# daisy9542/yolo-puncture

Hardware: AMD Instinct MI355X
Metric: images/sec (higher is better)
Workload: dtype bf16

## Files before the change

yolo-puncture_amd/csrc/conv_dwpw_stream.hip:

```cpp
#include "common.h"
#include <cstdlib>

namespace yp {

typedef __attribute__((ext_vector_type(8))) __bf16 bf16x8;
typedef __attribute__((ext_vector_type(4))) float f32x4;
typedef __attribute__((ext_vector_type(2))) float f32x2;
typedef __attribute__((address_space(3))) void lds_void;

constexpr int DS_TH = 8, DS_TW = 16;
constexpr int DS_C = 128;
constexpr int DS_HP = (DS_TH + 2) * (DS_TW + 2);
constexpr int DS_PIECES = 48;
constexpr int DS_HB = DS_PIECES * 1024;
constexpr int DS_AB = DS_TH * DS_TW * 256;

template <int N> __device__ __forceinline__ void ds_wait_vm() {
    static_assert(N >= 0 && N < 64, "vmcnt range");
    __builtin_amdgcn_s_waitcnt((N & 0xF) | (7 << 4) | (0xF << 8) | (((N >> 4) & 3) << 14));
}
__device__ __forceinline__ unsigned ds_lds_addr(const void* p) { return (unsigned)(size_t)(const __attribute__((address_space(3))) unsigned char*)p; }

template <int NW>
__global__ __launch_bounds__(NW * 64, 2) void conv_dwpw_stream_kernel(const DwPwParams p, const int tiles_h, const int tiles_w, const int num_tiles, const int G) {
    constexpr int RPW = DS_TH / NW;
    constexpr int NFW = 8 / NW;
    constexpr int NSLOT = NW == 8 ? 2 : 1;
    constexpr int NST = DS_TH * NFW;
    constexpr unsigned OOB = 0x80000000u;
    extern __shared__ __attribute__((aligned(1024))) unsigned char smem[];
    unsigned char* const Hs = smem;
    unsigned char* const As = smem + NSLOT * DS_HB;
    const int tid = threadIdx.x, lane = tid & 63;
    const int wave = __builtin_amdgcn_readfirstlane(tid >> 6);
    const int fr = lane & 15, fc = lane >> 4;

    const __amdgpu_buffer_rsrc_t xrs = __builtin_amdgcn_make_buffer_rsrc((void*)p.x, 0, (int)p.x_bytes, 0x00020000);
    const __amdgpu_buffer_rsrc_t wrs = __builtin_amdgcn_make_buffer_rsrc((void*)p.w_pw, 0, (int)p.wpw_bytes, 0x00020000);
    const __amdgpu_buffer_rsrc_t yrs = __builtin_amdgcn_make_buffer_rsrc((void*)p.y, 0, (int)p.y_bytes, 0x00020000);

    auto issue_tile = [&](int tile, int slot) {
        int t = tile;
        const int tw = t % tiles_w; t /= tiles_w;
        const int th = t % tiles_h;
        const int b = t / tiles_h;
        const int h0 = th * DS_TH - 1, w0 = tw * DS_TW - 1;
        unsigned char* const dst = Hs + slot * DS_HB;
#pragma unroll
        for (int j = 0; j < DS_PIECES / NW; ++j) {
            const int ii = wave + j * NW;
            const int s = ii * 64 + lane;
            const int hp = s >> 4, c = s & 15;
            const int hy = hp / (DS_TW + 2), hx = hp - hy * (DS_TW + 2);
            const int hi = h0 + hy, wi = w0 + hx;
            const bool ok = tile < num_tiles && hp < DS_HP && (unsigned)hi < (unsigned)p.H && (unsigned)wi < (unsigned)p.W;
            const unsigned voff = ok ? (unsigned)((((b * p.H + hi) * p.W + wi) * p.x_stride + p.x_coff + c * 8) * 2) : OOB;
            __builtin_amdgcn_raw_ptr_buffer_load_lds(xrs, (lds_void*)(dst + ii * 1024), 16, voff, 0, 0, 0);
        }
    };
    int tile = blockIdx.x;
    issue_tile(tile, 0);

    f32x2 wd[9], bd;
    {
        const unsigned* w32 = (const unsigned*)p.w_dw;
#pragma unroll
        for (int t = 0; t < 9; ++t) {
            const unsigned u = w32[t * (DS_C / 2) + lane];
            wd[t] = f32x2{__uint_as_float(u << 16), __uint_as_float(u & 0xffff0000u)};
        }
        bd = f32x2{p.b_dw[2 * lane], p.b_dw[2 * lane + 1]};
    }
    bf16x8 wreg[4][NFW];
    float bpw[NFW][4];
#pragma unroll
    for (int i = 0; i < NFW; ++i) {
#pragma unroll
        for (int ks = 0; ks < 4; ++ks) {
            const unsigned voff = (unsigned)((((wave * NFW + i) * 16 + fr) * p.Kpad + (ks >> 1) * 64 + fc * 16 + (ks & 1) * 8) * 2);
            const __attribute__((ext_vector_type(4))) unsigned v = __builtin_amdgcn_raw_buffer_load_b128(wrs, voff, 0, 0);
            wreg[ks][i] = __builtin_bit_cast(bf16x8, v);
        }
#pragma unroll
        for (int r = 0; r < 4; ++r) { const int co = (wave * NFW + i) * 16 + fc * 4 + r; bpw[i][r] = (co < p.Cout) ? p.b_pw[co] : 0.f; }
    }
    ds_wait_vm<0>();
#pragma unroll
    for (int t = 0; t < 9; ++t) asm volatile("" : "+v"(wd[t]));
    asm volatile("" : "+v"(bd));
#pragma unroll
    for (int i = 0; i < NFW; ++i) {
#pragma unroll
        for (int ks = 0; ks < 4; ++ks) asm volatile("" : "+v"(wreg[ks][i]));
#pragma unroll
        for (int r = 0; r < 4; ++r) asm volatile("" : "+v"(bpw[i][r]));
    }

    const unsigned as_l = ds_lds_addr(As);
    for (int it = 0; tile < num_tiles; tile += G, ++it) {
        if (it == 0) ds_wait_vm<0>();
        else ds_wait_vm<NST>();
        __builtin_amdgcn_s_barrier();
        const int slot = NSLOT == 2 ? (it & 1) : 0;
        if (NSLOT == 2) issue_tile(tile + G, slot ^ 1);
        int t = tile;
        const int tw = t % tiles_w; t /= tiles_w;
        const int th = t % tiles_h;
        const int b = t / tiles_h;
#pragma unroll
        for (int rr = 0; rr < RPW; ++rr) {
            const int row = wave * RPW + rr;
            f32x2 win[3][3];
            auto rd = [&](int ky, int col) -> f32x2 {
                const unsigned u = *(const unsigned*)(Hs + slot * DS_HB + ((row + ky) * (DS_TW + 2) + col) * 256 + lane * 4);
                return f32x2{__uint_as_float(u << 16), __uint_as_float(u & 0xffff0000u)};
            };
#pragma unroll
            for (int ky = 0; ky < 3; ++ky) { win[ky][0] = rd(ky, 0); win[ky][1] = rd(ky, 1); }
#pragma unroll
            for (int x = 0; x < DS_TW; ++x) {
#pragma unroll
                for (int ky = 0; ky < 3; ++ky) win[ky][2] = rd(ky, x + 2);
                f32x2 a = bd;
#pragma unroll
                for (int ky = 0; ky < 3; ++ky)
#pragma unroll
                    for (int kx = 0; kx < 3; ++kx) a = __builtin_elementwise_fma(win[ky][kx], wd[ky * 3 + kx], a);
                if (p.act_dw == ACT_SILU) {
                    f32x2 e = a * -1.4426950408889634f;
                    e[0] = __builtin_amdgcn_exp2f(e[0]); e[1] = __builtin_amdgcn_exp2f(e[1]);
                    e = e + 1.0f;
                    e[0] = __builtin_amdgcn_rcpf(e[0]); e[1] = __builtin_amdgcn_rcpf(e[1]);
                    a = a * e;
                }
                __attribute__((aligned(4))) __bf16 o[2] = {(__bf16)a[0], (__bf16)a[1]};
                const int px = row * DS_TW + x;
                const unsigned dst = as_l + (unsigned)(px * 256 + (((lane >> 2) ^ (px & 15)) << 4) + (lane & 3) * 4);
                asm volatile("ds_write_b32 %0, %1" : : "v"(dst), "v"(*(const unsigned*)o) : "memory");
#pragma unroll
                for (int ky = 0; ky < 3; ++ky) { win[ky][0] = win[ky][1]; win[ky][1] = win[ky][2]; }
            }
        }
        asm volatile("s_waitcnt lgkmcnt(0)" ::: "memory");
        __builtin_amdgcn_s_barrier();
        if (NSLOT == 1) issue_tile(tile + G, 0);
        f32x4 acc[NFW][DS_TH];
#pragma unroll
        for (int i = 0; i < NFW; ++i)
#pragma unroll
            for (int f = 0; f < DS_TH; ++f) acc[i][f] = f32x4{bpw[i][0], bpw[i][1], bpw[i][2], bpw[i][3]};
#pragma unroll
        for (int ks = 0; ks < 4; ++ks) {
            const int ch = (ks >> 1) * 8 + fc * 2 + (ks & 1);
            bf16x8 xf[DS_TH];
#pragma unroll
            for (int f = 0; f < DS_TH; ++f) xf[f] = *(const bf16x8*)(As + (f * 16 + fr) * 256 + ((ch ^ fr) << 4));
#pragma unroll
            for (int i = 0; i < NFW; ++i)
#pragma unroll
                for (int f = 0; f < DS_TH; ++f) acc[i][f] = __builtin_amdgcn_mfma_f32_16x16x32_bf16(wreg[ks][i], xf[f], acc[i][f], 0, 0, 0);
        }
        const int wo = tw * DS_TW + fr;
#pragma unroll
        for (int i = 0; i < NFW; ++i) {
            const int co = (wave * NFW + i) * 16 + fc * 4;
#pragma unroll
            for (int f = 0; f < DS_TH; ++f) {
                const int ho = th * DS_TH + f;
                const bool ok = ho < p.H && wo < p.W && co < p.Cout;
                float v[4] = {acc[i][f][0], acc[i][f][1], acc[i][f][2], acc[i][f][3]};
                if (p.act_pw == ACT_SILU) silu4_packed(v);
                __attribute__((aligned(8))) __bf16 o[4] = {(__bf16)v[0], (__bf16)v[1], (__bf16)v[2], (__bf16)v[3]};
                const unsigned off = ok ? (unsigned)((((b * p.H + ho) * p.W + wo) * p.y_stride + p.y_coff + co) * 2) : OOB;
                __builtin_amdgcn_raw_buffer_store_b64(*(const __attribute__((ext_vector_type(2))) unsigned*)o, yrs, off, 0, 0);
            }
        }
    }
    ds_wait_vm<0>();
}

bool dwpw_stream_valid(const DwPwParams& p) {
    static const bool off = [] { const char* v = std::getenv("YOLOP_NO_DWPW_STREAM"); return v && *v == '1'; }();
    if (off || p.w3 || p.out_f32 || p.clk) return false;
    if (p.C != DS_C || p.Kpad != DS_C || p.Cout != 128) return false;
    if ((p.x_stride & 7) || (p.x_coff & 7) || (p.y_stride & 3) || (p.y_coff & 3)) return false;
    if (p.x_bytes >= (1ull << 31) || p.y_bytes >= (1ull << 31) || p.wpw_bytes >= (1ull << 31)) return false;
    if (p.act_dw != ACT_SILU && p.act_dw != ACT_NONE) return false;
    if (p.act_pw != ACT_SILU && p.act_pw != ACT_NONE) return false;
    return (long)((p.H + DS_TH - 1) / DS_TH * DS_TH) * ((p.W + DS_TW - 1) / DS_TW * DS_TW) * 2 <= (long)p.H * p.W * 3;
}

template <int NW>
static hipError_t launch_dwpw_stream_t(const DwPwParams& p, hipStream_t st) {
    const size_t sh = (size_t)(NW == 8 ? 2 : 1) * DS_HB + DS_AB;
    auto kern = conv_dwpw_stream_kernel<NW>;
    static bool attr = false;
    if (!attr) {
        hipError_t e = hipFuncSetAttribute((const void*)kern, hipFuncAttributeMaxDynamicSharedMemorySize, 160 * 1024);
        if (e != hipSuccess) return e;
        attr = true;
    }
    const int tiles_h = (p.H + DS_TH - 1) / DS_TH, tiles_w = (p.W + DS_TW - 1) / DS_TW;
    const int num_tiles = p.B * tiles_h * tiles_w;
    const int gmax = NW == 8 ? 256 : 512;
    const int G = num_tiles < gmax ? num_tiles : gmax;
    hipLaunchKernelGGL(kern, dim3((unsigned)G), dim3(NW * 64), sh, st, p, tiles_h, tiles_w, num_tiles, G);
    return hipGetLastError();
}

hipError_t launch_dwpw_stream(const DwPwParams& p, hipStream_t st) {
    if (!dwpw_stream_valid(p)) return hipErrorInvalidValue;
    static const bool one = [] { const char* v = std::getenv("YOLOP_DWPW_STREAM_ONE"); return v && *v == '1'; }();
    return one ? launch_dwpw_stream_t<8>(p, st) : launch_dwpw_stream_t<4>(p, st);
}

}
```

Measured before the change: 22390.

## Software-pipeline depthwise stage with paired LDS reads and templated activations

Restructures the depthwise loop into unrolled 4-column groups. Halo reads are issued one group ahead with ds_read2st64 pairs and explicit lgkmcnt waits, so LDS latency overlaps the FMAs. Write addresses become compile-time offsets on a precomputed base, and the activation types become template parameters so the runtime branches disappear. It also adds an optional s_memtime clock instrumentation path. In exchange it carries more registers for double-buffered raw reads, and it relies on hand-counted waitcnt values being correct.

```diff
diff --git a/yolo-puncture_amd/csrc/conv_dwpw_stream.hip b/yolo-puncture_amd/csrc/conv_dwpw_stream.hip
--- a/yolo-puncture_amd/csrc/conv_dwpw_stream.hip
+++ b/yolo-puncture_amd/csrc/conv_dwpw_stream.hip
@@ -1,11 +1,16 @@
 #include "common.h"
+#include <cstdio>
 #include <cstdlib>
+#include <utility>
+#include <vector>
 
 namespace yp {
 
 typedef __attribute__((ext_vector_type(8))) __bf16 bf16x8;
 typedef __attribute__((ext_vector_type(4))) float f32x4;
 typedef __attribute__((ext_vector_type(2))) float f32x2;
+typedef __attribute__((ext_vector_type(2))) __bf16 bf16x2;
+typedef __attribute__((ext_vector_type(2))) unsigned u32x2;
 typedef __attribute__((address_space(3))) void lds_void;
 
 constexpr int DS_TH = 8, DS_TW = 16;
@@ -13,6 +18,7 @@
 constexpr int DS_HP = (DS_TH + 2) * (DS_TW + 2);
 constexpr int DS_PIECES = 48;
 constexpr int DS_HB = DS_PIECES * 1024;
+static_assert(DS_HB % 1024 == 0, "the depthwise stage's write swizzle is one XOR into address bits 4..7: every halo slot and the operand tile behind them must start 1-KiB aligned");
 constexpr int DS_AB = DS_TH * DS_TW * 256;
 
 template <int N> __device__ __forceinline__ void ds_wait_vm() {
@@ -21,12 +27,35 @@
 }
 __device__ __forceinline__ unsigned ds_lds_addr(const void* p) { return (unsigned)(size_t)(const __attribute__((address_space(3))) unsigned char*)p; }
 
-template <int NW>
+template <int P0, int P1> __device__ __forceinline__ void ds_rd2px(u32x2& d, unsigned a) {
+    static_assert(P0 >= 0 && P1 < 256, "ds_read2st64 offset range");
+    asm volatile("ds_read2st64_b32 %0, %1 offset0:%2 offset1:%3" : "=v"(d) : "v"(a), "n"(P0), "n"(P1));
+}
+template <int OFF> __device__ __forceinline__ void ds_wr32(unsigned a, unsigned v) {
+    static_assert(OFF >= 0 && OFF < 65536, "ds_write offset range");
+    asm volatile("ds_write_b32 %0, %1 offset:%2" : : "v"(a), "v"(v), "n"(OFF));
+}
+template <int N, bool FIRST> __device__ __forceinline__ void ds_wait_lgkm(u32x2 (&r)[3][3]) {
+    static_assert(N >= 0 && N < 16, "lgkmcnt range");
+    if (FIRST)
+        asm volatile("s_waitcnt lgkmcnt(%9)" : "+v"(r[0][0]), "+v"(r[0][1]), "+v"(r[0][2]), "+v"(r[1][0]), "+v"(r[1][1]), "+v"(r[1][2]),
+                                               "+v"(r[2][0]), "+v"(r[2][1]), "+v"(r[2][2]) : "n"(N));
+    else
+        asm volatile("s_waitcnt lgkmcnt(%6)" : "+v"(r[0][1]), "+v"(r[0][2]), "+v"(r[1][1]), "+v"(r[1][2]), "+v"(r[2][1]), "+v"(r[2][2]) : "n"(N));
+}
+template <int... I, class F> __device__ __forceinline__ void ds_static_for(std::integer_sequence<int, I...>, F&& f) { (f(std::integral_constant<int, I>{}), ...); }
+__device__ __forceinline__ unsigned ds_pk_bf16(float a, float b) {
+    return __builtin_bit_cast(unsigned, __builtin_convertvector(f32x2{a, b}, bf16x2));
+}
+
+template <int NW, int ADW, int APW, bool CLK>
 __global__ __launch_bounds__(NW * 64, 2) void conv_dwpw_stream_kernel(const DwPwParams p, const int tiles_h, const int tiles_w, const int num_tiles, const int G) {
     constexpr int RPW = DS_TH / NW;
     constexpr int NFW = 8 / NW;
     constexpr int NSLOT = NW == 8 ? 2 : 1;
     constexpr int NST = DS_TH * NFW;
+    constexpr int CG = 4;
+    constexpr int NU = RPW * (DS_TW / CG);
     constexpr unsigned OOB = 0x80000000u;
     extern __shared__ __attribute__((aligned(1024))) unsigned char smem[];
     unsigned char* const Hs = smem;
@@ -38,6 +67,12 @@
     const __amdgpu_buffer_rsrc_t xrs = __builtin_amdgcn_make_buffer_rsrc((void*)p.x, 0, (int)p.x_bytes, 0x00020000);
     const __amdgpu_buffer_rsrc_t wrs = __builtin_amdgcn_make_buffer_rsrc((void*)p.w_pw, 0, (int)p.wpw_bytes, 0x00020000);
     const __amdgpu_buffer_rsrc_t yrs = __builtin_amdgcn_make_buffer_rsrc((void*)p.y, 0, (int)p.y_bytes, 0x00020000);
+
+    unsigned long long clk[5] = {0, 0, 0, 0, 0};
+    unsigned long long last = 0;
+    auto stamp = [&](int i) {
+        if (CLK) { const unsigned long long now = __builtin_amdgcn_s_memtime(); clk[i] += now - last; last = now; }
+    };
 
     auto issue_tile = [&](int tile, int slot) {
         int t = tile;
@@ -96,53 +131,81 @@
         for (int r = 0; r < 4; ++r) asm volatile("" : "+v"(bpw[i][r]));
     }
 
-    const unsigned as_l = ds_lds_addr(As);
+    const unsigned hs_l = ds_lds_addr(Hs) + (unsigned)(wave * RPW * (DS_TW + 2) * 256 + lane * 4);
+    const unsigned aw_l = ds_lds_addr(As) + (unsigned)(wave * RPW * DS_TW * 256 + ((lane >> 2) << 4) + (lane & 3) * 4);
+    if (CLK) last = __builtin_amdgcn_s_memtime();
     for (int it = 0; tile < num_tiles; tile += G, ++it) {
-        if (it == 0) ds_wait_vm<0>();
-        else ds_wait_vm<NST>();
+        ds_wait_vm<NST>();
         __builtin_amdgcn_s_barrier();
+        stamp(0);
         const int slot = NSLOT == 2 ? (it & 1) : 0;
+        const unsigned hs_t = hs_l + (unsigned)(slot * DS_HB);
+        u32x2 raw[2][3][3];
+        auto rd = [&](auto U) {
+            constexpr int u = decltype(U)::value, rr = u / (DS_TW / CG), c0 = (u % (DS_TW / CG)) * CG;
+            ds_static_for(std::make_integer_sequence<int, 3>{}, [&](auto KY) {
+                constexpr int ky = decltype(KY)::value, px = (rr + ky) * (DS_TW + 2) + c0;
+                if (c0 == 0) ds_rd2px<px, px + 1>(raw[u & 1][ky][0], hs_t);
+                ds_rd2px<px + 2, px + 3>(raw[u & 1][ky][1], hs_t);
+                ds_rd2px<px + 4, px + 5>(raw[u & 1][ky][2], hs_t);
+            });
+        };
+        rd(std::integral_constant<int, 0>{});
         if (NSLOT == 2) issue_tile(tile + G, slot ^ 1);
         int t = tile;
         const int tw = t % tiles_w; t /= tiles_w;
         const int th = t % tiles_h;
         const int b = t / tiles_h;
-#pragma unroll
-        for (int rr = 0; rr < RPW; ++rr) {
-            const int row = wave * RPW + rr;
-            f32x2 win[3][3];
-            auto rd = [&](int ky, int col) -> f32x2 {
-                const unsigned u = *(const unsigned*)(Hs + slot * DS_HB + ((row + ky) * (DS_TW + 2) + col) * 256 + lane * 4);
-                return f32x2{__uint_as_float(u << 16), __uint_as_float(u & 0xffff0000u)};
-            };
-#pragma unroll
-            for (int ky = 0; ky < 3; ++ky) { win[ky][0] = rd(ky, 0); win[ky][1] = rd(ky, 1); }
-#pragma unroll
-            for (int x = 0; x < DS_TW; ++x) {
-#pragma unroll
-                for (int ky = 0; ky < 3; ++ky) win[ky][2] = rd(ky, x + 2);
-                f32x2 a = bd;
-#pragma unroll
-                for (int ky = 0; ky < 3; ++ky)
-#pragma unroll
-                    for (int kx = 0; kx < 3; ++kx) a = __builtin_elementwise_fma(win[ky][kx], wd[ky * 3 + kx], a);
-                if (p.act_dw == ACT_SILU) {
-                    f32x2 e = a * -1.4426950408889634f;
-                    e[0] = __builtin_amdgcn_exp2f(e[0]); e[1] = __builtin_amdgcn_exp2f(e[1]);
-                    e = e + 1.0f;
-                    e[0] = __builtin_amdgcn_rcpf(e[0]); e[1] = __builtin_amdgcn_rcpf(e[1]);
-                    a = a * e;
-                }
-                __attribute__((aligned(4))) __bf16 o[2] = {(__bf16)a[0], (__bf16)a[1]};
-                const int px = row * DS_TW + x;
-                const unsigned dst = as_l + (unsigned)(px * 256 + (((lane >> 2) ^ (px & 15)) << 4) + (lane & 3) * 4);
-                asm volatile("ds_write_b32 %0, %1" : : "v"(dst), "v"(*(const unsigned*)o) : "memory");
-#pragma unroll
-                for (int ky = 0; ky < 3; ++ky) { win[ky][0] = win[ky][1]; win[ky][1] = win[ky][2]; }
+        f32x2 car[3][2];
+        ds_static_for(std::make_integer_sequence<int, NU>{}, [&](auto U) {
+            constexpr int u = decltype(U)::value, rr = u / (DS_TW / CG), c0 = (u % (DS_TW / CG)) * CG;
+            constexpr bool first = c0 == 0, nfirst = (u + 1) % (DS_TW / CG) == 0;
+            if constexpr (u + 1 < NU) rd(std::integral_constant<int, u + 1>{});
+            ds_wait_lgkm<(u > 0 ? CG : 0) + (u + 1 < NU ? (nfirst ? 9 : 6) : 0), first>(raw[u & 1]);
+            f32x2 win[3][CG + 2];
+#pragma unroll
+            for (int ky = 0; ky < 3; ++ky) {
+#pragma unroll
+                for (int q = first ? 0 : 1; q < 3; ++q)
+#pragma unroll
+                    for (int h = 0; h < 2; ++h) {
+                        const unsigned v = raw[u & 1][ky][q][h];
+                        win[ky][2 * q + h] = f32x2{__uint_as_float(v << 16), __uint_as_float(v & 0xffff0000u)};
+                    }
+                if (!first) { win[ky][0] = car[ky][0]; win[ky][1] = car[ky][1]; }
+                car[ky][0] = win[ky][CG]; car[ky][1] = win[ky][CG + 1];
             }
-        }
+            f32x2 a[CG];
+#pragma unroll
+            for (int j = 0; j < CG; ++j) a[j] = bd;
+#pragma unroll
+            for (int ky = 0; ky < 3; ++ky)
+#pragma unroll
+                for (int kx = 0; kx < 3; ++kx)
+#pragma unroll
+                    for (int j = 0; j < CG; ++j) a[j] = __builtin_elementwise_fma(win[ky][j + kx], wd[ky * 3 + kx], a[j]);
+            if (ADW == ACT_SILU) {
+                f32x2 e[CG];
+#pragma unroll
+                for (int j = 0; j < CG; ++j) e[j] = a[j] * -1.4426950408889634f;
+#pragma unroll
+                for (int j = 0; j < CG; ++j) { e[j][0] = __builtin_amdgcn_exp2f(e[j][0]); e[j][1] = __builtin_amdgcn_exp2f(e[j][1]); }
+#pragma unroll
+                for (int j = 0; j < CG; ++j) e[j] = e[j] + 1.0f;
+#pragma unroll
+                for (int j = 0; j < CG; ++j) { e[j][0] = __builtin_amdgcn_rcpf(e[j][0]); e[j][1] = __builtin_amdgcn_rcpf(e[j][1]); }
+#pragma unroll
+                for (int j = 0; j < CG; ++j) a[j] = a[j] * e[j];
+            }
+            ds_static_for(std::make_integer_sequence<int, CG>{}, [&](auto J) {
+                constexpr int x = c0 + decltype(J)::value;
+                ds_wr32<(rr * DS_TW + x) * 256>(aw_l ^ (unsigned)(x << 4), ds_pk_bf16(a[decltype(J)::value][0], a[decltype(J)::value][1]));
+            });
+        });
         asm volatile("s_waitcnt lgkmcnt(0)" ::: "memory");
+        stamp(1);
         __builtin_amdgcn_s_barrier();
+        stamp(2);
         if (NSLOT == 1) issue_tile(tile + G, 0);
         f32x4 acc[NFW][DS_TH];
 #pragma unroll
@@ -160,6 +223,7 @@
 #pragma unroll
                 for (int f = 0; f < DS_TH; ++f) acc[i][f] = __builtin_amdgcn_mfma_f32_16x16x32_bf16(wreg[ks][i], xf[f], acc[i][f], 0, 0, 0);
         }
+        stamp(3);
         const int wo = tw * DS_TW + fr;
 #pragma unroll
         for (int i = 0; i < NFW; ++i) {
@@ -169,14 +233,16 @@
                 const int ho = th * DS_TH + f;
                 const bool ok = ho < p.H && wo < p.W && co < p.Cout;
                 float v[4] = {acc[i][f][0], acc[i][f][1], acc[i][f][2], acc[i][f][3]};
-                if (p.act_pw == ACT_SILU) silu4_packed(v);
-                __attribute__((aligned(8))) __bf16 o[4] = {(__bf16)v[0], (__bf16)v[1], (__bf16)v[2], (__bf16)v[3]};
+                if (APW == ACT_SILU) silu4_packed(v);
                 const unsigned off = ok ? (unsigned)((((b * p.H + ho) * p.W + wo) * p.y_stride + p.y_coff + co) * 2) : OOB;
-                __builtin_amdgcn_raw_buffer_store_b64(*(const __attribute__((ext_vector_type(2))) unsigned*)o, yrs, off, 0, 0);
+                __builtin_amdgcn_raw_buffer_store_b64(u32x2{ds_pk_bf16(v[0], v[1]), ds_pk_bf16(v[2], v[3])}, yrs, off, 0, 0);
             }
         }
+        stamp(4);
     }
     ds_wait_vm<0>();
+    if (CLK && lane == 0)
+        for (int i = 0; i < 5; ++i) p.clk[((size_t)blockIdx.x * NW + wave) * 5 + i] = clk[i];
 }
 
 bool dwpw_stream_valid(const DwPwParams& p) {
@@ -190,10 +256,10 @@
     return (long)((p.H + DS_TH - 1) / DS_TH * DS_TH) * ((p.W + DS_TW - 1) / DS_TW * DS_TW) * 2 <= (long)p.H * p.W * 3;
 }
 
-template <int NW>
+template <int NW, int ADW, int APW>
 static hipError_t launch_dwpw_stream_t(const DwPwParams& p, hipStream_t st) {
     const size_t sh = (size_t)(NW == 8 ? 2 : 1) * DS_HB + DS_AB;
-    auto kern = conv_dwpw_stream_kernel<NW>;
+    auto kern = conv_dwpw_stream_kernel<NW, ADW, APW, false>;
     static bool attr = false;
     if (!attr) {
         hipError_t e = hipFuncSetAttribute((const void*)kern, hipFuncAttributeMaxDynamicSharedMemorySize, 160 * 1024);
@@ -204,14 +270,51 @@
     const int num_tiles = p.B * tiles_h * tiles_w;
     const int gmax = NW == 8 ? 256 : 512;
     const int G = num_tiles < gmax ? num_tiles : gmax;
+    static const bool clocks = [] { const char* v = std::getenv("YOLOP_DWPW_STREAM_CLOCKS"); return v && *v == '1'; }();
+    if (clocks) {
+        hipStreamCaptureStatus cap = hipStreamCaptureStatusNone;
+        hipError_t e = hipStreamIsCapturing(st, &cap);
+        if (e != hipSuccess) return e;
+        if (cap != hipStreamCaptureStatusNone) return hipErrorStreamCaptureUnsupported;
+        auto kclk = conv_dwpw_stream_kernel<NW, ADW, APW, true>;
+        e = hipFuncSetAttribute((const void*)kclk, hipFuncAttributeMaxDynamicSharedMemorySize, 160 * 1024);
+        if (e != hipSuccess) return e;
+        DwPwParams q = p;
+        const size_t n = (size_t)G * NW * 5;
+        e = hipMalloc((void**)&q.clk, n * 8);
+        if (e != hipSuccess) return e;
+        std::vector<unsigned long long> h(n);
+        hipLaunchKernelGGL(kclk, dim3((unsigned)G), dim3(NW * 64), sh, st, q, tiles_h, tiles_w, num_tiles, G);
+        e = hipGetLastError();
+        if (e == hipSuccess) e = hipStreamSynchronize(st);
+        if (e == hipSuccess) e = hipMemcpy(h.data(), q.clk, n * 8, hipMemcpyDeviceToHost);
+        (void)hipFree(q.clk);
+        if (e != hipSuccess) return e;
+        static const char* nm[5] = {"wait+barrier(a)", "depthwise", "barrier(b)", "pointwise", "epilogue"};
+        const double tiles = (double)num_tiles / G;
+        fprintf(stderr, "[dwpw stream clocks] NW=%d %dx%d B=%d, s_memtime ticks per wave and tile (mean over waves):", NW, p.H, p.W, p.B);
+        for (int i = 0; i < 5; ++i) {
+            double s = 0;
+            for (size_t g = 0; g < (size_t)G * NW; ++g) s += (double)h[g * 5 + i];
+            fprintf(stderr, " %s %.0f", nm[i], s / ((double)G * NW) / tiles);
+        }
+        fprintf(stderr, "\n");
+        return hipSuccess;
+    }
     hipLaunchKernelGGL(kern, dim3((unsigned)G), dim3(NW * 64), sh, st, p, tiles_h, tiles_w, num_tiles, G);
     return hipGetLastError();
+}
+
+template <int NW>
+static hipError_t launch_dwpw_stream_nw(const DwPwParams& p, hipStream_t st) {
+    if (p.act_dw == ACT_SILU) return p.act_pw == ACT_SILU ? launch_dwpw_stream_t<NW, ACT_SILU, ACT_SILU>(p, st) : launch_dwpw_stream_t<NW, ACT_SILU, ACT_NONE>(p, st);
+    return p.act_pw == ACT_SILU ? launch_dwpw_stream_t<NW, ACT_NONE, ACT_SILU>(p, st) : launch_dwpw_stream_t<NW, ACT_NONE, ACT_NONE>(p, st);
 }
 
 hipError_t launch_dwpw_stream(const DwPwParams& p, hipStream_t st) {
     if (!dwpw_stream_valid(p)) return hipErrorInvalidValue;
     static const bool one = [] { const char* v = std::getenv("YOLOP_DWPW_STREAM_ONE"); return v && *v == '1'; }();
-    return one ? launch_dwpw_stream_t<8>(p, st) : launch_dwpw_stream_t<4>(p, st);
-}
-
-}
+    return one ? launch_dwpw_stream_nw<8>(p, st) : launch_dwpw_stream_nw<4>(p, st);
+}
+
+}
```

Measured after the change: 22550, median of 6. About the same (+0.7%).
